# singhhp1069/charon

Hardware: AMD Instinct MI355X
Metric: verified+aggregated 3-of-4 threshold BLS sigs/sec at 1/2/4/8 MI355X (higher is better)
Workload: dtype u32 (Fp 14x28-bit limbs); 1 GPU; config2: 3-of-4, 10000 DVs x 1 attestation per GPU; parallelism=shard1, inflight_launches=3, batches_per_launch=16, rlc_group=16, rlc_chunk=8, gident=0, subgroup_batch=0, level0=passed, hw_queues=4

## Files before the change

### charon_amd/_native.py

```python
from __future__ import annotations

import ctypes
import os
import shutil
import subprocess

PKG = os.path.dirname(os.path.abspath(__file__))
ROOT = os.path.dirname(PKG)
CSRC = os.path.join(PKG, "csrc")
LIB_PATH = os.path.join(PKG, "libtbls_gpu.so")
HEADER = os.path.join(ROOT, "include", "tbls_gpu.h")
HEADERS = [HEADER, os.path.join(ROOT, "include", "tbls_ssz.h")]


def _hipcc():
    for c in ("/opt/rocm/bin/hipcc", shutil.which("hipcc") or ""):
        if c and os.path.exists(c):
            return c
    raise RuntimeError("hipcc not found: cannot build libtbls_gpu.so")


def _clangxx():
    c = "/opt/rocm/llvm/bin/clang++"
    if not os.path.exists(c):
# ... 169 lines not shown
    "tbg_submit_sets": (ctypes.c_int, [ctypes.c_void_p, ctypes.POINTER(TbgBatch), ctypes.c_void_p, ctypes.c_uint32,
                                       ctypes.POINTER(ctypes.c_uint64)]),
    "tbg_collect_sets": (ctypes.c_int, [ctypes.c_void_p, ctypes.c_uint64, ctypes.c_void_p, ctypes.c_void_p,
                                        ctypes.c_int]),
    "tbg_fetch_sets": (ctypes.c_int, [ctypes.c_void_p, ctypes.c_uint64, ctypes.c_void_p, ctypes.c_void_p]),
    "tbg_run": (ctypes.c_int, [ctypes.c_void_p, ctypes.POINTER(TbgBatch), ctypes.c_void_p, ctypes.c_void_p,
                               ctypes.c_void_p]),
    "tbg_replay": (ctypes.c_int, [ctypes.c_void_p, ctypes.c_uint64, ctypes.c_uint32, ctypes.c_void_p]),
    "tbg_replay_multi": (ctypes.c_int, [ctypes.c_void_p, ctypes.c_void_p, ctypes.c_uint32, ctypes.c_uint32,
                                        ctypes.c_void_p]),
    "tbg_fetch": (ctypes.c_int, [ctypes.c_void_p, ctypes.c_uint64, ctypes.c_void_p, ctypes.c_void_p, ctypes.c_void_p]),
    "tbg_fetch_stats": (ctypes.c_int, [ctypes.c_void_p, ctypes.c_uint64, ctypes.c_void_p]),
    "tbg_fetch_level0": (ctypes.c_int, [ctypes.c_void_p, ctypes.c_uint64, ctypes.c_void_p]),
    "tbg_fetch_fallback": (ctypes.c_int, [ctypes.c_void_p, ctypes.c_uint64, ctypes.c_void_p]),
    "tbg_fetch_subgroup": (ctypes.c_int, [ctypes.c_void_p, ctypes.c_uint64, ctypes.c_void_p]),
    "tbg_fetch_shape": (ctypes.c_int, [ctypes.c_void_p, ctypes.c_uint64, ctypes.c_void_p]),
    "tbg_host_stats": (ctypes.c_int, [ctypes.c_void_p, ctypes.c_void_p, ctypes.c_int]),
    "tbg_multi_host_stats": (ctypes.c_int, [ctypes.c_void_p, ctypes.c_void_p, ctypes.c_int]),
    "tbg_slot_bytes": (ctypes.c_int, [ctypes.c_void_p, ctypes.c_uint64, ctypes.c_void_p, ctypes.c_void_p]),
    "tbg_last_timings": (ctypes.c_int, [ctypes.c_void_p, ctypes.c_void_p]),
    "tbg_sk_to_pk": (ctypes.c_int, [ctypes.c_void_p, ctypes.c_void_p, ctypes.c_uint32, ctypes.c_void_p]),
    "tbg_sign": (ctypes.c_int, [ctypes.c_void_p, ctypes.c_void_p, ctypes.c_uint32, ctypes.c_void_p, ctypes.c_void_p,
                                ctypes.c_uint32, ctypes.c_void_p, ctypes.c_void_p]),
    "tbg_poll": (ctypes.c_int, [ctypes.c_void_p, ctypes.c_uint64]),
    "tbg_submit_group": (ctypes.c_int, [ctypes.c_void_p, ctypes.c_void_p, ctypes.c_uint32, ctypes.c_void_p]),
    "tbg_replay_profile": (ctypes.c_int, [ctypes.c_void_p, ctypes.c_uint64, ctypes.c_void_p, ctypes.c_uint32,
                                          ctypes.POINTER(ctypes.c_uint32)]),
    "tbg_replay_plan": (ctypes.c_int, [ctypes.c_void_p, ctypes.c_void_p, ctypes.c_void_p, ctypes.c_uint32,
                                       ctypes.c_void_p]),
    "tbg_multi_init": (ctypes.c_int, [ctypes.POINTER(TbgConfig), ctypes.c_void_p, ctypes.c_uint32,
# ... 21 lines not shown
    "tbg_signing_roots": (ctypes.c_int, [ctypes.c_uint32, ctypes.c_char_p, ctypes.c_uint32, ctypes.c_char_p,
                                         ctypes.c_uint32, ctypes.c_void_p, ctypes.c_void_p, ctypes.c_uint32]),
}

_lib = None


def load() -> ctypes.CDLL:
    global _lib
    if _lib is None:
        path = os.environ.get("TBG_LIB", LIB_PATH)
        if not os.path.exists(path):
            raise RuntimeError(f"{path} is missing: run __graft_entry__.build() (hipcc, gfx950)")
        lib = ctypes.CDLL(path)
        for name, (res, args) in SIGNATURES.items():
            fn = getattr(lib, name)
            fn.restype = res
            fn.argtypes = args
        _lib = lib
    return _lib
```

### charon_amd/csrc/bls_sgb.h

```cpp
#pragma once
#include "bls_pair.h"

namespace tbg {

template <class F, bool FAST>
TBG_HD Jac<F> sgb_add_g(const Jac<F>& p, const Jac<F>& q, bool& exc) {
  if constexpr (FAST) return jac_add_x(p, q, exc);
  else return jac_add(p, q);
}

template <class F, bool FAST, class L>
TBG_HD Jac<F> sgb_fold_g(L&& slice, uint32_t n_slices, bool& exc) {
  Jac<F> acc = slice(0u);
#pragma unroll 1
  for (uint32_t sl = 1; sl < n_slices; ++sl) acc = sgb_add_g<F, FAST>(acc, slice(sl), exc);
  return acc;
}

template <class F, bool FAST, class L>
TBG_HD Jac<F> sgb_running_sums_g(L&& bucket, uint32_t n_v, bool& exc) {
  Jac<F> run = jac_inf<F>(), q = run;
#pragma unroll 1
  for (int v = (int)n_v; v >= 1; --v) {
    run = sgb_add_g<F, FAST>(run, bucket((uint32_t)(v - 1)), exc);
    q = sgb_add_g<F, FAST>(q, run, exc);
  }
  return q;
}

}
```

### charon_amd/csrc/k_msm.hip

```cpp
#define TBG_ADD_DBL_INLINE 1
#ifndef TBG_SCHED_FENCE
#define TBG_SCHED_FENCE 1
#endif
#include "tbls_launch.h"
#include "bls_msm.h"
#include "bls_pair.h"
#include "bls_batchinv.h"

namespace tbg {

__global__ void __launch_bounds__(BINV_BLOCK) k_pubkey_tables(const G1A* pk, const G1A* xpk, const int32_t* status,
                                                              uint32_t n, G1A* tab) {
  const uint32_t i = blockIdx.x * blockDim.x + threadIdx.x;
  const bool in = i < n;
  const bool ok = in && status[i] == DEC_OK;
  G1A p0{fp_zero(), fp_zero()}, x0 = p0;
  if (ok) {
    p0 = pk[i];
    x0 = xpk[i];
  }
#if TBG_PK_W2
#pragma unroll 1
  for (int k = 0; k < (int)PK_TAB; ++k) {
    const G1J e = ok ? rlc_key_table_w2_entry(p0, x0, k) : jac_inf<Fp>();
// ... 212 lines not shown
  px_store(*B.batch_pt, Aff<Fp2x>{f_mul(acc.X, zi2), f_mul(acc.Y, f_mul(zi2, zi))});
}

__global__ void __launch_bounds__(2 * L0F_PAIRS) k_l0f_reduce(DevBatch B, uint32_t n_sg, uint32_t wq, uint32_t n_t) {
  __shared__ Jac<Fp2x> lds[2 * L0F_PAIRS];
  if (B.counters[CNT_L0_BAD]) return;
  const uint32_t pr = threadIdx.x >> 1, b = blockIdx.x;
  const bool qcol = b < SGB_K * wq;
  const uint32_t col = qcol ? b / wq : SGB_K, chunk = qcol ? b % wq : b - SGB_K * wq;
  const uint32_t count = qcol ? n_sg : n_sg * n_t;
  const uint32_t a0 = chunk * L0F_CHUNK + pr * L0F_PER, a1 = min(a0 + L0F_PER, count);
  Jac<Fp2x> acc = jac_inf<Fp2x>();
#pragma unroll 1
  for (uint32_t a = a0; a < a1; ++a) {
    if (qcol) {
      acc = jac_add_in<Fp2x, true>(acc, px_load(B.sgb_part[((size_t)SGB_BUCKETS * a + (size_t)SGB_V * col) * B.sgb_split]));
    } else {
      acc = jac_add_in<Fp2x, true>(acc, px_load(B.sgb_t[a]));
    }
  }
  acc = pair_tree_sum<L0F_PAIRS>(acc, lds);
  if (pr == 0) px_store(B.l0f_sum[b], acc);
}

__global__ void __launch_bounds__(2 * L0F_PAIRS) k_l0f_fold(DevBatch B, uint32_t wq, uint32_t wt) {
  TBG_URGENT();
  __shared__ Jac<Fp2x> lds[2 * L0F_PAIRS];
  if (B.counters[CNT_L0_BAD]) return;
  const uint32_t pr = threadIdx.x >> 1, col = blockIdx.x;
  const uint32_t first = col < SGB_K ? col * wq : SGB_K * wq, count = col < SGB_K ? wq : wt;
  Jac<Fp2x> acc = jac_inf<Fp2x>();
// ... 57 lines not shown
```

### charon_amd/csrc/k_sgb.hip

```cpp
#define TBG_ADD_DBL_INLINE 1
#ifndef TBG_SCHED_FENCE
#define TBG_SCHED_FENCE 1
#endif
#include "tbls_launch.h"
#include "bls_rlc.h"
#include "bls_sgb.h"

namespace tbg {

#ifndef TBG_SGB_SORT_BLOCK
#define TBG_SGB_SORT_BLOCK 256
#endif
constexpr uint32_t kSgbSortBlock = TBG_SGB_SORT_BLOCK;

__global__ void __launch_bounds__(kSgbSortBlock) k_sgb_sort(DevBatch B) {
  __shared__ uint32_t cnt[SGB_BUCKETS];
  __shared__ uint32_t off[SGB_BUCKETS + 1];
  __shared__ int8_t dig[SGB_M * SGB_K];
  const uint32_t g = blockIdx.x, t = threadIdx.x, m = B.sgb_m;
  const uint32_t i0 = g * m;
  const uint32_t n = min(m, B.n_partials - i0);
  for (uint32_t b = t; b < SGB_BUCKETS; b += kSgbSortBlock) cnt[b] = 0;
  if (t == 0) B.sgb_bad[g] = 0;
  const bool fused = l0_fused(B);
  __syncthreads();
  for (uint32_t li = t; li < n; li += kSgbSortBlock) {
    const bool ok = B.partial_status[i0 + li] == TBG_PS_NOT_VERIFIED;
    int32_t c[SGB_K];
    sgb_digits(B.sgb_seed, i0 + li, c);
    if (fused) {
      uint32_t u[4];
      l0f_digits(c, u);
      *(uint4*)(B.l0f_u + 4ull * (i0 + li)) = make_uint4(u[0], u[1], u[2], u[3]);
    }
#pragma unroll
    for (uint32_t k = 0; k < SGB_K; ++k) {
      const int32_t d = ok ? c[k] : 0;
      dig[li * SGB_K + k] = (int8_t)d;
      if (d) atomicAdd(&cnt[k * SGB_V + (uint32_t)(d < 0 ? -d : d) - 1], 1u);
    }
  }
  __syncthreads();
  if (t == 0) {
    uint32_t run = 0;
    for (uint32_t b = 0; b < SGB_BUCKETS; ++b) {
      off[b] = run;
      run += cnt[b];
    }
    off[SGB_BUCKETS] = run;
  }
// ... 5 lines not shown
  }
  __syncthreads();
  uint32_t* ent = B.sgb_ent + (size_t)m * SGB_K * g;
  for (uint32_t li = t; li < n; li += kSgbSortBlock) {
#pragma unroll 1
    for (uint32_t k = 0; k < SGB_K; ++k) {
      const int32_t d = dig[li * SGB_K + k];
      if (!d) continue;
      const uint32_t pos = atomicAdd(&cnt[k * SGB_V + (uint32_t)(d < 0 ? -d : d) - 1], 1u);
      ent[pos] = (li << 1) | (d < 0 ? 1u : 0u);
    }
  }
}

__global__ void TBG_LAUNCH_N(TBG_PAIR_WAVES) k_sgb_bucket(DevBatch B, uint32_t n_sg, uint32_t n_t) {
  const uint32_t w = (blockIdx.x * blockDim.x + threadIdx.x) >> 1;
  const uint32_t S = B.sgb_split, m = B.sgb_m;
  if (w >= n_sg * SGB_BUCKETS * S) {
    const uint32_t wt = w - n_sg * SGB_BUCKETS * S;
    if (wt >= n_sg * n_t) return;
    const uint32_t i0 = (wt / n_t) * m + (wt % n_t) * SGB_T_PER;
    const uint32_t i1 = min(min(i0 + SGB_T_PER, (wt / n_t + 1) * m), B.n_partials);
    Jac<Fp2x> acc = jac_inf<Fp2x>();
#pragma unroll 1
    for (uint32_t i = i0; i < i1; ++i) {
      if (B.partial_status[i] != TBG_PS_NOT_VERIFIED) continue;
      Aff<Fp2x> p = px_load(B.sig_aff[i]);
      p.y = f_reduce(p.y);
      acc = jac_add_aff_in(acc, p);
    }
    px_store(B.sgb_t[wt], acc);
    return;
  }
  const uint32_t g = w / (SGB_BUCKETS * S), b = (w / S) % SGB_BUCKETS, sl = w % S;
  const uint32_t* goff = B.sgb_off + (size_t)(SGB_BUCKETS + 1) * g;
  const uint32_t o0 = goff[b], n = goff[b + 1] - o0;
  const uint32_t e0 = o0 + (n * sl) / S, e1 = o0 + (n * (sl + 1)) / S;
  const uint32_t* ent = B.sgb_ent + (size_t)m * SGB_K * g;
  const G2A* sig = B.sig_aff + (size_t)m * g;
  Jac<Fp2x> acc = jac_inf<Fp2x>();
#pragma unroll 1
  for (uint32_t e = e0; e < e1; ++e) {
    const uint32_t v = ent[e];
    Aff<Fp2x> p = px_load(sig[v >> 1]);
    p.y = f_reduce(p.y);
    if (v & 1u) p.y = f_reduce(f_neg(p.y));
    acc = jac_add_aff_in(acc, p);
  }
  px_store(B.sgb_part[w], acc);
}

__device__ __forceinline__ void sgb_fail(const DevBatch& B, uint32_t g) {
  B.sgb_bad[g] = 1u;
  if (l0_fused(B)) B.counters[CNT_L0_BAD] = 1u;
}

__device__ __noinline__ Jac<Fp2x> sgb_fold_complete(const G2J* part, uint32_t S) {
  bool unused = false;
  return sgb_fold_g<Fp2x, false>([&](uint32_t sl) { return px_load(part[sl]); }, S, unused);
}

__global__ void TBG_LAUNCH_N(TBG_PAIR_WAVES) k_sgb_fold(DevBatch B, uint32_t n_sg) {
  const uint32_t w = (blockIdx.x * blockDim.x + threadIdx.x) >> 1;
  if (w >= n_sg * SGB_BUCKETS) return;
  const uint32_t S = B.sgb_split;
  G2J* part = B.sgb_part + (size_t)w * S;
  bool exc = false;
  Jac<Fp2x> acc = sgb_fold_g<Fp2x, true>([&](uint32_t sl) { return px_load(part[sl]); }, S, exc);
  if (!pair_all(!exc)) acc = sgb_fold_complete(part, S);
  px_store(part[0], acc);
}

__device__ __noinline__ Jac<Fp2x> sgb_combine_complete(const G2J* part, uint32_t S) {
  bool unused = false;
  return sgb_running_sums_g<Fp2x, false>([&](uint32_t v) { return px_load(part[(size_t)v * S]); }, SGB_V, unused);
}

__global__ void TBG_LAUNCH_N(TBG_PAIR_WAVES) k_sgb_combine(DevBatch B, uint32_t n_sg) {
  const uint32_t w = (blockIdx.x * blockDim.x + threadIdx.x) >> 1;
  if (w >= n_sg * SGB_K) return;
  const uint32_t g = w / SGB_K, k = w % SGB_K, S = B.sgb_split;
  G2J* part = B.sgb_part + ((size_t)SGB_BUCKETS * g + (size_t)SGB_V * k) * S;
  bool exc = false;
  Jac<Fp2x> q = sgb_running_sums_g<Fp2x, true>([&](uint32_t v) { return px_load(part[(size_t)v * S]); }, SGB_V, exc);
  if (!pair_all(!exc)) q = sgb_combine_complete(part, S);
  px_store(part[0], q);
}

__global__ void TBG_LAUNCH_N(TBG_PAIR_WAVES) k_sgb_test(DevBatch B, uint32_t n_sg) {
  const uint32_t w = (blockIdx.x * blockDim.x + threadIdx.x) >> 1;
  if (w >= n_sg * SGB_K) return;
  const uint32_t g = w / SGB_K, k = w % SGB_K;
  const G2J& slot = B.sgb_part[((size_t)SGB_BUCKETS * g + (size_t)SGB_V * k) * B.sgb_split];
  bool ok = true;
  if (!jac_is_inf(px_load(slot))) {
    bool exc = false;
    Jac<Fp2x> m = px_load(slot);
#pragma unroll 1
    for (int i = 62; i >= 0; --i) {
      m = jac_dbl_lo(m);
      if ((X_ABS >> i) & 1) {
        __asm__ __volatile__("" ::: "memory");
        m = jac_add_x(m, px_load(slot), exc);
      }
    }
    if (exc || jac_is_inf(m)) {
      ok = false;
    } else {
// ... 1 lines not shown
      const Jac<Fp2x> ps = g2_psi_g(px_load(slot));
      const Fp2x z1 = f_sqr(ps.Z), z2 = f_sqr(m.Z);
      ok = f_eq(f_mul(ps.X, z2), f_mul(m.X, z1)) &&
           f_eq(f_mul(f_mul(ps.Y, m.Z), z2), f_reduce(f_neg(f_mul(f_mul(m.Y, ps.Z), z1))));
    }
  }
  if (!ok && pair_par() == 0) sgb_fail(B, g);
}

void launch_subgroup_batch(const DevBatch& B, hipStream_t st) {
  if (!B.sgb) return;
  const uint32_t n_sg = sgb_groups(B.n_partials, B.sgb_m);
  if (!n_sg) return;
  TBG_KLAUNCH(k_sgb_sort, dim3(n_sg), dim3(kSgbSortBlock), st, B);
  const uint32_t n_t = l0_fused(B) ? sgb_t_slices(B.sgb_m) : 0u;
  TBG_KLAUNCH(k_sgb_bucket, grid_for(2 * n_sg * (SGB_BUCKETS * B.sgb_split + n_t)), dim3(kBlock), st, B, n_sg, n_t);
  if (B.sgb_split > 1) TBG_KLAUNCH(k_sgb_fold, grid_for(2 * n_sg * SGB_BUCKETS), dim3(kBlock), st, B, n_sg);
  TBG_KLAUNCH(k_sgb_combine, grid_for(2 * n_sg * SGB_K), dim3(kBlock), st, B, n_sg);
  TBG_KLAUNCH(k_sgb_test, grid_for(2 * n_sg * SGB_K), dim3(kBlock), st, B, n_sg);
}

}
```

### charon_amd/csrc/tbls_engine.hip

```cpp
#include <hip/hip_runtime.h>
#include <cstdio>
#include <cstdlib>
#include <cstring>
#include <cmath>
#include <functional>
#include <algorithm>
#include <atomic>
#include <chrono>
#include <mutex>
#include <new>
#include <random>
#include <thread>
#include <vector>
#include "tbls_launch.h"
#include "bls_lines.h"

using namespace tbg;

namespace tbg {
void debug_after_launch(const char* kernel, hipStream_t st) {
  static const bool on = getenv("TBG_DEBUG_SYNC") && getenv("TBG_DEBUG_SYNC")[0] == '1';
  if (!on) return;
  hipEvent_t a;
  (void)hipEventCreate(&a);
// ... 642 lines not shown
  size_t w_bf = sec(l0 ? 4ull * 3 * 4 * NL : 0);
  size_t w_gf = sec(l0 ? 4ull * 3 * 4 * NL * grp_f_entries(ng) : 0);
  const bool gm = TBG_GMSM && G != 0;
  size_t w_gmoff = sec(gm ? 4ull * (GM_BUCKETS + 1) * ng : 0);
  size_t w_gment = sec(gm ? 64ull * np : 0);
  size_t w_gmpart = sec(gm ? sizeof(G2J) * GM_BUCKETS * (size_t)ng : 0);
  size_t w_gmlead = sec(gm ? 4ull * ng : 0);
  size_t w_gmlist = sec(gm ? 4ull * np : 0);
  size_t w_gmhist = sec(gm ? 4ull * 256 : 0);
  size_t w_gmorder = sec(gm ? 4ull * GM_BUCKETS * ng : 0);
  uint32_t sgb_m = SGB_M;
  const bool sgb = np >= SGB_MIN_PARTIALS && c->sgb_mode != TBG_SGB_OFF &&
                   (sgb_plan(c->nonsub_ema, sgb_m) || c->sgb_mode == TBG_SGB_ON);
  const uint32_t sgb_split = sgb_split_for(sgb_m);
  const size_t n_sg = sgb ? sgb_groups(np, sgb_m) : 0;
  size_t w_sgoff = sec(4ull * (SGB_BUCKETS + 1) * n_sg);
  size_t w_sgent = sec(4ull * sgb_m * SGB_K * n_sg);
  size_t w_sgpart = sec(sizeof(G2J) * SGB_BUCKETS * sgb_split * n_sg);
  size_t w_sgbad = sec(4ull * n_sg);
  const bool fused = l0 && sgb && TBG_PK_W2;
  const bool msm = l0 && !fused;
  size_t w_mr = sec(msm ? 8ull * np : 0);
  size_t w_moff = sec(msm ? 4ull * (MSM_BUCKETS + 1) : 0);
  size_t w_mcur = sec(msm ? 4ull * MSM_BUCKETS : 0);
  size_t w_ment = sec(msm ? 16ull * np : 0);
  size_t w_mbkt = sec(msm ? sizeof(G2J) * (size_t)MSM_BUCKETS : 0);
  size_t w_mpart = sec(msm ? sizeof(G2J) * (size_t)MSM_BUCKETS * MSM_SPLIT : 0);
  size_t w_msum = sec(msm ? sizeof(G2J) * (size_t)MSM_SUM_ENTRIES : 0);
  size_t w_sgt = sec(fused ? sizeof(G2J) * sgb_t_slices(sgb_m) * n_sg : 0);
  size_t w_l0fsum = sec(fused ? sizeof(G2J) * (size_t)l0f_sum_entries((uint32_t)n_sg, sgb_m) : 0);
  size_t w_l0fu = sec(fused ? 16ull * np : 0);
  size_t w_aacc = sec(op != TBG_OP_VERIFY ? sizeof(G2J) * (size_t)nd : 0);
  size_t w_alist = sec(op != TBG_OP_VERIFY ? 4ull * nd : 0);
// ... 218 lines not shown
  B.batch_f = (uint32_t*)(dw + w_bf);
  B.grp_f = (uint32_t*)(dw + w_gf);
  B.gm_off = (uint32_t*)(dw + w_gmoff);
  B.gm_ent = (uint32_t*)(dw + w_gment);
  B.gm_part = (G2J*)(dw + w_gmpart);
  B.gm_lead = (uint32_t*)(dw + w_gmlead);
  B.gm_list = (uint32_t*)(dw + w_gmlist);
  B.gm_hist = (uint32_t*)(dw + w_gmhist);
  B.gm_order = (uint32_t*)(dw + w_gmorder);
  B.sgb = sgb ? 1u : 0u;
  B.sgb_m = sgb_m;
  B.sgb_split = sgb_split;
  B.sgb_off = (uint32_t*)(dw + w_sgoff);
  B.sgb_ent = (uint32_t*)(dw + w_sgent);
  B.sgb_part = (G2J*)(dw + w_sgpart);
  B.sgb_bad = (uint32_t*)(dw + w_sgbad);
  B.sgb_t = (G2J*)(dw + w_sgt);
  B.l0f_sum = (G2J*)(dw + w_l0fsum);
  B.l0f_u = (uint32_t*)(dw + w_l0fu);
  B.agg_acc = (G2J*)(dw + w_aacc);
  B.agg_list = (uint32_t*)(dw + w_alist);

  hipStream_t st = s->st;
  if (hipStreamWaitEvent(st, c->keys_ready, 0) != hipSuccess ||
      hipMemcpyAsync(s->d_in, s->h_in, in_bytes, hipMemcpyHostToDevice, st) != hipSuccess)
    return release(TBG_E_DEVICE);
  rc = launch_chain(c, *s, B, s->ev);
  if (rc != TBG_OK) return release(rc);
  if (hipMemcpyAsync(s->h_out, dw + w_out, out_bytes, hipMemcpyDeviceToHost, st) != hipSuccess ||
      hipEventRecord(s->done, st) != hipSuccess)
// ... 356 lines not shown
int tbg_fetch_subgroup(tbg_ctx* c, tbg_ticket t, uint32_t* out3) {
  if (!c || !out3) return TBG_E_INVALID_ARG;
  std::lock_guard<std::mutex> lk(c->mu);
  Slot* s = find_ticket(c, t, false, nullptr);
  if (!s) return TBG_E_TICKET;
  HIP_TRY(hipSetDevice(c->device));
  out3[0] = out3[1] = out3[2] = 0;
  if (!s->last.sgb) return TBG_OK;
  out3[2] = s->last.sgb_m;
  const uint32_t n_sg = sgb_groups(s->last.n_partials, s->last.sgb_m);
  std::vector<uint32_t> bad(n_sg);
  HIP_TRY(hipMemcpyAsync(bad.data(), s->last.sgb_bad, 4ull * n_sg, hipMemcpyDeviceToHost, s->st));
  HIP_TRY(hipStreamSynchronize(s->st));
  out3[0] = n_sg;
  for (uint32_t g = 0; g < n_sg; ++g) out3[1] += bad[g] ? 1u : 0u;
  return TBG_OK;
}

int tbg_host_stats(tbg_ctx* c, uint64_t* out8, int reset) {
  if (!c || !out8) return TBG_E_INVALID_ARG;
  for (int k = 0; k < 8; ++k) out8[k] = reset ? c->host[k].exchange(0) : c->host[k].load();
  return TBG_OK;
}

int tbg_slot_bytes(tbg_ctx* c, tbg_ticket t, uint64_t* device_bytes, uint64_t* pinned_bytes) {
  if (!c || !device_bytes || !pinned_bytes) return TBG_E_INVALID_ARG;
  std::lock_guard<std::mutex> lk(c->mu);
  Slot* s = find_ticket(c, t, false, nullptr);
  if (!s) return TBG_E_TICKET;
  *device_bytes = (uint64_t)s->d_in_cap + (uint64_t)s->d_work_cap;
// ... 305 lines not shown
```

### charon_amd/csrc/tbls_launch.h

```cpp
#pragma once
#include <hip/hip_runtime.h>
#include "bls_curve.h"
#include "bls_lines.h"
#include "../../include/tbls_gpu.h"

namespace tbg {

constexpr int kBlock = 64;
#ifndef TBG_PK_W2
#define TBG_PK_W2 1
#endif
constexpr uint32_t PK_TAB = TBG_PK_W2 ? 8u : 2u;
#ifndef TBG_REPLAY_SHAPE
#define TBG_REPLAY_SHAPE 1
#endif
#ifndef TBG_L0_SHAPE
#define TBG_L0_SHAPE 1
#endif
#ifndef TBG_L0_SHAPE_WIDE
#define TBG_L0_SHAPE_WIDE 1
#endif
#ifndef TBG_FB_WINDOW
#define TBG_FB_WINDOW 32768u
#endif
// ... 83 lines not shown
  uint32_t* grp_f;
  uint32_t* gm_off;
  uint32_t* gm_ent;
  G2J* gm_part;
  uint32_t* gm_lead;
  uint32_t* gm_list;
  uint32_t* gm_hist;
  uint32_t* gm_order;
  uint32_t sgb;
  uint32_t sgb_m;
  uint32_t sgb_split;
  uint32_t sgb_seed[8];
  uint32_t* sgb_off;
  uint32_t* sgb_ent;
  G2J* sgb_part;
  uint32_t* sgb_bad;
  G2J* sgb_t;
  G2J* l0f_sum;
  uint32_t* l0f_u;
  G2J* agg_acc;
  uint32_t* agg_list;
  int32_t* partial_status;
  int32_t* duty_status;
  uint8_t* agg;
  uint32_t sets;
  uint32_t n_sets;
  const uint32_t* duty_set;
  int32_t* set_status;
};
enum SetTail : int { SET_BAD = 0, SET_ANY = 1, SET_TAIL = 2 };
// ... 12 lines not shown
#endif
#ifndef TBG_SGB_SPLIT
#define TBG_SGB_SPLIT 4
#endif
constexpr uint32_t SGB_M = TBG_SGB_M;
constexpr uint32_t SGB_M_MIN = 64;
constexpr uint32_t SGB_K = 18;
constexpr uint32_t SGB_V = 6;
constexpr uint32_t SGB_BUCKETS = SGB_K * SGB_V;
constexpr uint32_t SGB_SPLIT = TBG_SGB_SPLIT;
constexpr uint32_t SGB_MIN_PARTIALS = 2 * SGB_M;
TBG_HD uint32_t sgb_groups(uint32_t n_partials, uint32_t m) { return (n_partials + m - 1) / m; }
TBG_HD uint32_t sgb_split_for(uint32_t m) {
  const uint32_t s = SGB_SPLIT * m / SGB_M;
  return s ? s : 1u;
}
TBG_HD bool l0_fused(const DevBatch& B) {
  return TBG_PK_W2 && B.rlc_batch && B.rlc_group && B.sgb && B.n_partials;
}
constexpr uint32_t SGB_T_PER = 32;
TBG_HD uint32_t sgb_t_slices(uint32_t m) { return m / SGB_T_PER; }
constexpr uint32_t L0F_COLS = SGB_K + 1;
constexpr uint32_t L0F_PAIRS = 128, L0F_PER = 4;
constexpr uint32_t L0F_CHUNK = L0F_PAIRS * L0F_PER;
TBG_HD uint32_t l0f_q_chunks(uint32_t n_sg) { return (n_sg + L0F_CHUNK - 1) / L0F_CHUNK; }
TBG_HD uint32_t l0f_t_chunks(uint32_t n_sg, uint32_t m) { return (n_sg * sgb_t_slices(m) + L0F_CHUNK - 1) / L0F_CHUNK; }
TBG_HD uint32_t l0f_sum_entries(uint32_t n_sg, uint32_t m) {
  return SGB_K * l0f_q_chunks(n_sg) + l0f_t_chunks(n_sg, m) + L0F_COLS;
}
constexpr uint32_t L0_TREE_FAN = 4;
// ... 102 lines not shown
```

### charon_amd/engine.py

```python
from __future__ import annotations

import ctypes
import itertools
from dataclasses import dataclass

import numpy as np

from . import _native

PS_INVALID, PS_VALID, PS_NOT_VERIFIED = 0, 1, 2
PS_ERR_FLAGS, PS_ERR_FIELD, PS_ERR_CURVE, PS_ERR_SUBGROUP, PS_ERR_IDENTITY, PS_ERR_PUBKEY = -1, -2, -3, -4, -5, -6
DS_OK, DS_NOT_AGGREGATED = 0, 1
DS_INSUFFICIENT, DS_INSUFFICIENT_VALID = -20, -21
DS_AGG_TOO_FEW, DS_AGG_DUPLICATE_ID, DS_AGG_IDENTITY, DS_DECODE = -22, -23, -24, -25
SS_ERROR, SS_INVALID, SS_VALID = 30, 31, 32
OP_VERIFY, OP_AGGREGATE, OP_VERIFY_AGGREGATE = 1, 2, 3
NO_PUBKEY = 0xFFFFFFFF
TIMING_KEYS = ["decode", "hash", "combine", "h_lines", "verify", "lagrange", "aggregate", "total"]
VERIFY_RLC, VERIFY_EACH = 0, 1
RLC_L0_AUTO, RLC_L0_ON, RLC_L0_OFF = 0, 1, 2
GIDENT_OFF, GIDENT_L3, GIDENT_CHUNKS = 0, 1, 2
SGB_AUTO, SGB_ON, SGB_OFF = 0, 1, 2
EXPRESS_OFF = 0xFFFFFFFF
L0_NOT_RUN, L0_PASSED, L0_FAILED = 0, 1, 2
HOST_STAT_KEYS = ["submits", "partials_submitted", "pack_ns", "enqueue_ns", "collects", "partials_collected",
                  "gather_ns", "wait_ns"]
MULTI_HOST_STAT_KEYS = ["submits", "partials", "build_ns", "submit_wall_ns", "collects", "collect_wall_ns"] + \
    ["ctx_" + k for k in HOST_STAT_KEYS] + ["contexts", "reserved"]
E_PENDING = -6
E_INVALID_ARG, E_TICKET = -1, -7


class EngineError(RuntimeError):
    pass


def _ptr(a):
# ... 222 lines not shown
        out = np.zeros(4, dtype=np.uint32)
        self._check(self._lib.tbg_fetch_stats(self._h, ticket, _ptr(out)), "tbg_fetch_stats")
        return dict(zip(["groups", "duty_checks", "partial_checks", "group_size"], out.tolist()))

    def fallback(self, ticket) -> dict:
        out = np.zeros(8, dtype=np.uint32)
        self._check(self._lib.tbg_fetch_fallback(self._h, ticket, _ptr(out)), "tbg_fetch_fallback")
        return dict(zip(["groups", "group_searches", "chunks", "chunk_searches", "duty_searches", "partial_checks",
                         "group_size", "level0"], out.tolist()))

    def shape(self, ticket) -> dict:
        out = np.zeros(4, dtype=np.uint32)
        self._check(self._lib.tbg_fetch_shape(self._h, ticket, _ptr(out)), "tbg_fetch_shape")
        return dict(zip(["group", "chunk", "level0", "chunks"], out.tolist()))

    def subgroup(self, ticket) -> dict:
        out = np.zeros(3, dtype=np.uint32)
        self._check(self._lib.tbg_fetch_subgroup(self._h, ticket, _ptr(out)), "tbg_fetch_subgroup")
        return dict(zip(["groups", "failed", "group_size"], out.tolist()))

    def host_stats(self, reset=False) -> dict:
        out = np.zeros(8, dtype=np.uint64)
        self._check(self._lib.tbg_host_stats(self._h, _ptr(out), 1 if reset else 0), "tbg_host_stats")
        return dict(zip(HOST_STAT_KEYS, out.tolist()))

    def slot_bytes(self, ticket) -> tuple:
        dev, pin = ctypes.c_uint64(), ctypes.c_uint64()
        self._check(self._lib.tbg_slot_bytes(self._h, ticket, ctypes.byref(dev), ctypes.byref(pin)), "tbg_slot_bytes")
        return dev.value, pin.value

    def level0(self, ticket) -> int:
        st = ctypes.c_int32(0)
        self._check(self._lib.tbg_fetch_level0(self._h, ticket, ctypes.byref(st)), "tbg_fetch_level0")
        return st.value
# ... 183 lines not shown
```

### include/tbls_gpu.h

```cpp
#ifndef TBLS_GPU_H
#define TBLS_GPU_H

#include <stddef.h>
#include <stdint.h>

#ifdef __cplusplus
extern "C" {
#endif

#define TBG_OK 0
#define TBG_E_INVALID_ARG (-1)
#define TBG_E_DEVICE (-2)
#define TBG_E_OOM (-3)
#define TBG_E_NO_DEVICE (-4)
#define TBG_E_BUSY (-5)
#define TBG_E_PENDING (-6)
#define TBG_E_TICKET (-7)

#define TBG_PS_INVALID 0
#define TBG_PS_VALID 1
#define TBG_PS_NOT_VERIFIED 2
#define TBG_PS_ERR_FLAGS (-1)
#define TBG_PS_ERR_FIELD (-2)
#define TBG_PS_ERR_CURVE (-3)
// ... 110 lines not shown

int tbg_replay(tbg_ctx* ctx, tbg_ticket ticket, uint32_t iters, float* ms8);
int tbg_replay_multi(tbg_ctx* ctx, const tbg_ticket* tickets, uint32_t n_tickets, uint32_t iters, float* ms8);
int tbg_replay_plan(tbg_ctx* ctx, const tbg_ticket* tickets, const uint32_t* n_parts, uint32_t n_launches, float* ms8);
int tbg_fetch(tbg_ctx* ctx, tbg_ticket ticket, int32_t* partial_status, int32_t* duty_status, uint8_t* agg96);
typedef struct {
  char name[64];
  float ms;
} tbg_kernel_time;
int tbg_replay_profile(tbg_ctx* ctx, tbg_ticket ticket, tbg_kernel_time* out, uint32_t max_entries,
                       uint32_t* n_entries);
int tbg_fetch_stats(tbg_ctx* ctx, tbg_ticket ticket, uint32_t* out4);
int tbg_fetch_level0(tbg_ctx* ctx, tbg_ticket ticket, int32_t* state);
int tbg_fetch_fallback(tbg_ctx* ctx, tbg_ticket ticket, uint32_t* out8);
int tbg_fetch_subgroup(tbg_ctx* ctx, tbg_ticket ticket, uint32_t* out3);
int tbg_fetch_shape(tbg_ctx* ctx, tbg_ticket ticket, uint32_t* out4);
int tbg_host_stats(tbg_ctx* ctx, uint64_t* out8, int reset);
int tbg_slot_bytes(tbg_ctx* ctx, tbg_ticket ticket, uint64_t* device_bytes, uint64_t* pinned_bytes);

int tbg_sum_pubkeys(tbg_ctx* ctx, const uint32_t* pubkey_ids, const uint32_t* off, uint32_t n_sets, uint8_t* out48,
                    int32_t* status);
int tbg_sum_sigs(tbg_ctx* ctx, const uint8_t* sigs96, const uint32_t* off, uint32_t n_sets, uint8_t* out96,
                 int32_t* status, int32_t* sig_status);
int tbg_fast_aggregate_verify(tbg_ctx* ctx, const uint32_t* pubkey_ids, const uint32_t* key_off, uint32_t n_sets,
                              const uint8_t* msgs, const uint32_t* msg_off, const uint8_t* sigs96, int32_t* status);

int tbg_sk_to_pk(tbg_ctx* ctx, const uint8_t* sk32, uint32_t n, uint8_t* pk48);
int tbg_sign(tbg_ctx* ctx, const uint8_t* sk32, uint32_t n, const uint8_t* msgs, const uint32_t* msg_off,
             uint32_t n_msgs, const uint32_t* item_msg, uint8_t* sig96);

// ... 20 lines not shown
```

Before: 3.454 million DV-duties/s (n verifies + 1 aggregate each).

## Add paired-digit subgroup bucket schedule with count-ranked bucket dispatch

For subgroup sizes of at least 256, signed digits are combined in pairs into joint buckets, which roughly halves the number of bucket entries per partial. Bucket workers are dispatched in order of bucket occupancy so waves get similar amounts of work. A fold kernel rebuilds the per-digit bucket sums from the pair buckets. The cost is more buckets, extra fold additions, and more sort logic. A query that reports which schedule ran is also added.

Measured after the change: 3.573 million DV-duties/s (n verifies + 1 aggregate each), median of 6. 1.03x the previous value.

```diff
diff --git a/charon_amd/_native.py b/charon_amd/_native.py
--- a/charon_amd/_native.py
+++ b/charon_amd/_native.py
@@ -207,6 +207,7 @@
     "tbg_fetch_level0": (ctypes.c_int, [ctypes.c_void_p, ctypes.c_uint64, ctypes.c_void_p]),
     "tbg_fetch_fallback": (ctypes.c_int, [ctypes.c_void_p, ctypes.c_uint64, ctypes.c_void_p]),
     "tbg_fetch_subgroup": (ctypes.c_int, [ctypes.c_void_p, ctypes.c_uint64, ctypes.c_void_p]),
+    "tbg_fetch_subgroup_schedule": (ctypes.c_int, [ctypes.c_void_p, ctypes.c_uint64, ctypes.c_void_p]),
     "tbg_fetch_shape": (ctypes.c_int, [ctypes.c_void_p, ctypes.c_uint64, ctypes.c_void_p]),
     "tbg_host_stats": (ctypes.c_int, [ctypes.c_void_p, ctypes.c_void_p, ctypes.c_int]),
     "tbg_multi_host_stats": (ctypes.c_int, [ctypes.c_void_p, ctypes.c_void_p, ctypes.c_int]),
@@ -258,7 +259,11 @@
             raise RuntimeError(f"{path} is missing: run __graft_entry__.build() (hipcc, gfx950)")
         lib = ctypes.CDLL(path)
         for name, (res, args) in SIGNATURES.items():
-            fn = getattr(lib, name)
+            fn = getattr(lib, name, None)
+            if fn is None:
+                if path == LIB_PATH:
+                    raise RuntimeError(f"{path} does not export {name}: rebuild it (__graft_entry__.build())")
+                continue
             fn.restype = res
             fn.argtypes = args
         _lib = lib
diff --git a/charon_amd/csrc/bls_sgb.h b/charon_amd/csrc/bls_sgb.h
--- a/charon_amd/csrc/bls_sgb.h
+++ b/charon_amd/csrc/bls_sgb.h
@@ -28,4 +28,38 @@
   return q;
 }
 
+constexpr uint32_t SGBP_V = 6;
+constexpr uint32_t SGBP_ROW = 2 * SGBP_V + 1;
+constexpr uint32_t SGBP_B = SGBP_V + SGBP_V * SGBP_ROW;
+constexpr uint32_t SGBP_SUMS = 2 * SGBP_V;
+constexpr uint32_t SGBP_NONE = 0xFFu;
+TBG_HD uint32_t sgb_pair_index(uint32_t a, int32_t b) {
+  return a ? SGBP_V + (a - 1) * SGBP_ROW + (uint32_t)(b + (int32_t)SGBP_V) : (uint32_t)b - 1;
 }
+TBG_HD uint32_t sgb_pair_code(int32_t c0, int32_t c1) {
+  if (!c0 && !c1) return SGBP_NONE;
+  const bool neg = c0 < 0 || (!c0 && c1 < 0);
+  return sgb_pair_index((uint32_t)(neg ? -c0 : c0), neg ? -c1 : c1) | (neg ? 0x80u : 0u);
+}
+template <class F, bool FAST, class L>
+TBG_HD Jac<F> sgb_pair_sum_g(L&& bucket, uint32_t j, bool& exc) {
+  Jac<F> acc = jac_inf<F>();
+#pragma unroll 1
+  for (uint32_t t = 0; t < SGBP_ROW; ++t) {
+    uint32_t idx;
+    bool neg = false;
+    if (j < SGBP_V) {
+      idx = sgb_pair_index(j + 1, (int32_t)t - (int32_t)SGBP_V);
+    } else {
+      const int32_t v = (int32_t)(j - SGBP_V) + 1;
+      neg = t > SGBP_V;
+      idx = t == 0 ? sgb_pair_index(0, v) : sgb_pair_index(neg ? t - SGBP_V : t, neg ? -v : v);
+    }
+    Jac<F> x = bucket(idx);
+    if (neg) x = jac_neg(x);
+    acc = sgb_add_g<F, FAST>(acc, x, exc);
+  }
+  return acc;
+}
+
+}
diff --git a/charon_amd/csrc/k_msm.hip b/charon_amd/csrc/k_msm.hip
--- a/charon_amd/csrc/k_msm.hip
+++ b/charon_amd/csrc/k_msm.hip
@@ -250,7 +250,7 @@
 #pragma unroll 1
   for (uint32_t a = a0; a < a1; ++a) {
     if (qcol) {
-      acc = jac_add_in<Fp2x, true>(acc, px_load(B.sgb_part[((size_t)SGB_BUCKETS * a + (size_t)SGB_V * col) * B.sgb_split]));
+      acc = jac_add_in<Fp2x, true>(acc, px_load(B.sgb_part[sgb_q_slot(B, a, col)]));
     } else {
       acc = jac_add_in<Fp2x, true>(acc, px_load(B.sgb_t[a]));
     }
diff --git a/charon_amd/csrc/k_sgb.hip b/charon_amd/csrc/k_sgb.hip
--- a/charon_amd/csrc/k_sgb.hip
+++ b/charon_amd/csrc/k_sgb.hip
@@ -13,14 +13,51 @@
 #endif
 constexpr uint32_t kSgbSortBlock = TBG_SGB_SORT_BLOCK;
 
-__global__ void __launch_bounds__(kSgbSortBlock) k_sgb_sort(DevBatch B) {
-  __shared__ uint32_t cnt[SGB_BUCKETS];
-  __shared__ uint32_t off[SGB_BUCKETS + 1];
-  __shared__ int8_t dig[SGB_M * SGB_K];
+static_assert(SGBP_B == SGB_PB && SGBP_V == SGB_V && SGBP_SUMS * SGB_PAIRS == SGB_BUCKETS, "bls_sgb.h's pair layout");
+static_assert((kSgbSortBlock & (kSgbSortBlock - 1)) == 0, "sgb_block_scan: a power of two");
+constexpr uint32_t SGB_RANK_KEYS = 256;
+
+template <uint32_t N>
+__device__ __forceinline__ void sgb_block_scan(uint32_t* a, uint32_t* tmp) {
+  constexpr uint32_t PER = (N + kSgbSortBlock - 1) / kSgbSortBlock;
+  const uint32_t t = threadIdx.x, b0 = t * PER;
+  uint32_t sum = 0;
+  for (uint32_t j = 0; j < PER; ++j)
+    if (b0 + j < N) sum += a[b0 + j];
+  tmp[t] = sum;
+  __syncthreads();
+  for (uint32_t d = 1; d < kSgbSortBlock; d <<= 1) {
+    const uint32_t x = t >= d ? tmp[t - d] : 0u;
+    __syncthreads();
+    tmp[t] += x;
+    __syncthreads();
+  }
+  uint32_t run = tmp[t] - sum;
+  for (uint32_t j = 0; j < PER; ++j)
+    if (b0 + j < N) {
+      const uint32_t x = a[b0 + j];
+      a[b0 + j] = run;
+      run += x;
+    }
+  if (t == kSgbSortBlock - 1) a[N] = tmp[t];
+  __syncthreads();
+}
+
+__device__ __forceinline__ void sgb_sort_paired(const DevBatch& B, uint8_t* lds) {
+  uint8_t* code = lds;
+  uint32_t* cnt = (uint32_t*)(lds + SGB_M * SGB_PAIRS);
+  uint32_t* hist = cnt + SGB_PBUCKETS + 1;
+  uint32_t* tmp = hist + SGB_RANK_KEYS + 1;
+  uint8_t* key = (uint8_t*)(tmp + kSgbSortBlock);
+  static_assert((SGB_M * SGB_PAIRS) % 4 == 0 &&
+                    SGB_M * SGB_PAIRS + 4 * (SGB_PBUCKETS + 1 + SGB_RANK_KEYS + 1 + kSgbSortBlock) + SGB_PBUCKETS <=
+                        SGB_M * SGB_K,
+                "the paired sort's arrays fit the digit array");
   const uint32_t g = blockIdx.x, t = threadIdx.x, m = B.sgb_m;
   const uint32_t i0 = g * m;
   const uint32_t n = min(m, B.n_partials - i0);
-  for (uint32_t b = t; b < SGB_BUCKETS; b += kSgbSortBlock) cnt[b] = 0;
+  for (uint32_t b = t; b < SGB_PBUCKETS; b += kSgbSortBlock) cnt[b] = 0;
+  for (uint32_t b = t; b < SGB_RANK_KEYS; b += kSgbSortBlock) hist[b] = 0;
   if (t == 0) B.sgb_bad[g] = 0;
   const bool fused = l0_fused(B);
   __syncthreads();
@@ -34,6 +71,65 @@
       *(uint4*)(B.l0f_u + 4ull * (i0 + li)) = make_uint4(u[0], u[1], u[2], u[3]);
     }
 #pragma unroll
+    for (uint32_t p = 0; p < SGB_PAIRS; ++p) {
+      const uint32_t cd = ok ? sgb_pair_code(c[2 * p], c[2 * p + 1]) : SGBP_NONE;
+      code[li * SGB_PAIRS + p] = (uint8_t)cd;
+      if (cd != SGBP_NONE) atomicAdd(&cnt[p * SGB_PB + (cd & 0x7Fu)], 1u);
+    }
+  }
+  __syncthreads();
+  for (uint32_t b = t; b < SGB_PBUCKETS; b += kSgbSortBlock) {
+    const uint32_t k = SGB_RANK_KEYS - 1 - min(cnt[b], SGB_RANK_KEYS - 1);
+    key[b] = (uint8_t)k;
+    atomicAdd(&hist[k], 1u);
+  }
+  __syncthreads();
+  sgb_block_scan<SGB_PBUCKETS>(cnt, tmp);
+  sgb_block_scan<SGB_RANK_KEYS>(hist, tmp);
+  uint32_t* goff = B.sgb_off + (size_t)(SGB_PBUCKETS + 1) * g;
+  uint32_t* rank = B.sgb_rank + (size_t)SGB_PBUCKETS * g;
+  for (uint32_t b = t; b <= SGB_PBUCKETS; b += kSgbSortBlock) {
+    goff[b] = cnt[b];
+    if (b < SGB_PBUCKETS) rank[atomicAdd(&hist[key[b]], 1u)] = b;
+  }
+  __syncthreads();
+  uint32_t* ent = B.sgb_ent + (size_t)sgb_ent_stride(m) * g;
+  for (uint32_t li = t; li < n; li += kSgbSortBlock) {
+#pragma unroll 1
+    for (uint32_t p = 0; p < SGB_PAIRS; ++p) {
+      const uint32_t cd = code[li * SGB_PAIRS + p];
+      if (cd == SGBP_NONE) continue;
+      const uint32_t pos = atomicAdd(&cnt[p * SGB_PB + (cd & 0x7Fu)], 1u);
+      ent[pos] = (li << 1) | (cd >> 7);
+    }
+  }
+}
+
+__global__ void __launch_bounds__(kSgbSortBlock) k_sgb_sort(DevBatch B) {
+  __shared__ uint32_t cnt[SGB_BUCKETS];
+  __shared__ uint32_t off[SGB_BUCKETS + 1];
+  __shared__ __attribute__((aligned(16))) int8_t dig[SGB_M * SGB_K];
+  if (sgb_paired(B.sgb_m)) {
+    sgb_sort_paired(B, (uint8_t*)dig);
+    return;
+  }
+  const uint32_t g = blockIdx.x, t = threadIdx.x, m = B.sgb_m;
+  const uint32_t i0 = g * m;
+  const uint32_t n = min(m, B.n_partials - i0);
+  for (uint32_t b = t; b < SGB_BUCKETS; b += kSgbSortBlock) cnt[b] = 0;
+  if (t == 0) B.sgb_bad[g] = 0;
+  const bool fused = l0_fused(B);
+  __syncthreads();
+  for (uint32_t li = t; li < n; li += kSgbSortBlock) {
+    const bool ok = B.partial_status[i0 + li] == TBG_PS_NOT_VERIFIED;
+    int32_t c[SGB_K];
+    sgb_digits(B.sgb_seed, i0 + li, c);
+    if (fused) {
+      uint32_t u[4];
+      l0f_digits(c, u);
+      *(uint4*)(B.l0f_u + 4ull * (i0 + li)) = make_uint4(u[0], u[1], u[2], u[3]);
+    }
+#pragma unroll
     for (uint32_t k = 0; k < SGB_K; ++k) {
       const int32_t d = ok ? c[k] : 0;
       dig[li * SGB_K + k] = (int8_t)d;
@@ -69,10 +165,13 @@
 }
 
 __global__ void TBG_LAUNCH_N(TBG_PAIR_WAVES) k_sgb_bucket(DevBatch B, uint32_t n_sg, uint32_t n_t) {
-  const uint32_t w = (blockIdx.x * blockDim.x + threadIdx.x) >> 1;
+  uint32_t w = (blockIdx.x * blockDim.x + threadIdx.x) >> 1;
   const uint32_t S = B.sgb_split, m = B.sgb_m;
-  if (w >= n_sg * SGB_BUCKETS * S) {
-    const uint32_t wt = w - n_sg * SGB_BUCKETS * S;
+  const bool paired = sgb_paired(m);
+  const uint32_t per_g = paired ? SGB_PRANK : SGB_BUCKETS * S;
+  const bool is_t = paired ? w < n_sg * n_t : w >= n_sg * per_g;
+  if (is_t) {
+    const uint32_t wt = paired ? w : w - n_sg * per_g;
     if (wt >= n_sg * n_t) return;
     const uint32_t i0 = (wt / n_t) * m + (wt % n_t) * SGB_T_PER;
     const uint32_t i1 = min(min(i0 + SGB_T_PER, (wt / n_t + 1) * m), B.n_partials);
@@ -87,11 +186,28 @@
     px_store(B.sgb_t[wt], acc);
     return;
   }
-  const uint32_t g = w / (SGB_BUCKETS * S), b = (w / S) % SGB_BUCKETS, sl = w % S;
-  const uint32_t* goff = B.sgb_off + (size_t)(SGB_BUCKETS + 1) * g;
-  const uint32_t o0 = goff[b], n = goff[b + 1] - o0;
-  const uint32_t e0 = o0 + (n * sl) / S, e1 = o0 + (n * (sl + 1)) / S;
-  const uint32_t* ent = B.sgb_ent + (size_t)m * SGB_K * g;
+  if (paired) w -= n_sg * n_t;
+  if (w >= n_sg * per_g) return;
+  const uint32_t g = w / per_g;
+  uint32_t e0, e1;
+  size_t out;
+  if (paired) {
+    const uint32_t r = w % SGB_PRANK;
+    if (r >= SGB_PBUCKETS) return;
+    const uint32_t b = B.sgb_rank[(size_t)SGB_PBUCKETS * g + r];
+    const uint32_t* goff = B.sgb_off + (size_t)(SGB_PBUCKETS + 1) * g;
+    e0 = goff[b];
+    e1 = goff[b + 1];
+    out = (size_t)sgb_part_stride(m) * g + b;
+  } else {
+    const uint32_t b = (w / S) % SGB_BUCKETS, sl = w % S;
+    const uint32_t* goff = B.sgb_off + (size_t)(SGB_BUCKETS + 1) * g;
+    const uint32_t o0 = goff[b], n = goff[b + 1] - o0;
+    e0 = o0 + (n * sl) / S;
+    e1 = o0 + (n * (sl + 1)) / S;
+    out = w;
+  }
+  const uint32_t* ent = B.sgb_ent + (size_t)sgb_ent_stride(m) * g;
   const G2A* sig = B.sig_aff + (size_t)m * g;
   Jac<Fp2x> acc = jac_inf<Fp2x>();
 #pragma unroll 1
@@ -102,7 +218,7 @@
     if (v & 1u) p.y = f_reduce(f_neg(p.y));
     acc = jac_add_aff_in(acc, p);
   }
-  px_store(B.sgb_part[w], acc);
+  px_store(B.sgb_part[out], acc);
 }
 
 __device__ __forceinline__ void sgb_fail(const DevBatch& B, uint32_t g) {
@@ -115,9 +231,24 @@
   return sgb_fold_g<Fp2x, false>([&](uint32_t sl) { return px_load(part[sl]); }, S, unused);
 }
 
+__device__ __noinline__ Jac<Fp2x> sgb_pair_sum_complete(const G2J* bk, uint32_t j) {
+  bool unused = false;
+  return sgb_pair_sum_g<Fp2x, false>([&](uint32_t idx) { return px_load(bk[idx]); }, j, unused);
+}
+
 __global__ void TBG_LAUNCH_N(TBG_PAIR_WAVES) k_sgb_fold(DevBatch B, uint32_t n_sg) {
   const uint32_t w = (blockIdx.x * blockDim.x + threadIdx.x) >> 1;
   if (w >= n_sg * SGB_BUCKETS) return;
+  if (sgb_paired(B.sgb_m)) {
+    const uint32_t g = w / SGB_BUCKETS, p = (w % SGB_BUCKETS) / SGBP_SUMS, j = w % SGBP_SUMS;
+    G2J* grp = B.sgb_part + (size_t)sgb_part_stride(B.sgb_m) * g;
+    const G2J* bk = grp + (size_t)SGB_PB * p;
+    bool exc = false;
+    Jac<Fp2x> acc = sgb_pair_sum_g<Fp2x, true>([&](uint32_t idx) { return px_load(bk[idx]); }, j, exc);
+    if (!pair_all(!exc)) acc = sgb_pair_sum_complete(bk, j);
+    px_store(grp[SGB_PBUCKETS + w % SGB_BUCKETS], acc);
+    return;
+  }
   const uint32_t S = B.sgb_split;
   G2J* part = B.sgb_part + (size_t)w * S;
   bool exc = false;
@@ -134,8 +265,8 @@
 __global__ void TBG_LAUNCH_N(TBG_PAIR_WAVES) k_sgb_combine(DevBatch B, uint32_t n_sg) {
   const uint32_t w = (blockIdx.x * blockDim.x + threadIdx.x) >> 1;
   if (w >= n_sg * SGB_K) return;
-  const uint32_t g = w / SGB_K, k = w % SGB_K, S = B.sgb_split;
-  G2J* part = B.sgb_part + ((size_t)SGB_BUCKETS * g + (size_t)SGB_V * k) * S;
+  const uint32_t g = w / SGB_K, k = w % SGB_K, S = sgb_paired(B.sgb_m) ? 1u : B.sgb_split;
+  G2J* part = B.sgb_part + sgb_q_slot(B, g, k);
   bool exc = false;
   Jac<Fp2x> q = sgb_running_sums_g<Fp2x, true>([&](uint32_t v) { return px_load(part[(size_t)v * S]); }, SGB_V, exc);
   if (!pair_all(!exc)) q = sgb_combine_complete(part, S);
@@ -146,7 +277,7 @@
   const uint32_t w = (blockIdx.x * blockDim.x + threadIdx.x) >> 1;
   if (w >= n_sg * SGB_K) return;
   const uint32_t g = w / SGB_K, k = w % SGB_K;
-  const G2J& slot = B.sgb_part[((size_t)SGB_BUCKETS * g + (size_t)SGB_V * k) * B.sgb_split];
+  const G2J& slot = B.sgb_part[sgb_q_slot(B, g, k)];
   bool ok = true;
   if (!jac_is_inf(px_load(slot))) {
     bool exc = false;
@@ -178,8 +309,10 @@
   if (!n_sg) return;
   TBG_KLAUNCH(k_sgb_sort, dim3(n_sg), dim3(kSgbSortBlock), st, B);
   const uint32_t n_t = l0_fused(B) ? sgb_t_slices(B.sgb_m) : 0u;
-  TBG_KLAUNCH(k_sgb_bucket, grid_for(2 * n_sg * (SGB_BUCKETS * B.sgb_split + n_t)), dim3(kBlock), st, B, n_sg, n_t);
-  if (B.sgb_split > 1) TBG_KLAUNCH(k_sgb_fold, grid_for(2 * n_sg * SGB_BUCKETS), dim3(kBlock), st, B, n_sg);
+  const bool paired = sgb_paired(B.sgb_m);
+  const uint32_t per_g = paired ? SGB_PRANK : SGB_BUCKETS * B.sgb_split;
+  TBG_KLAUNCH(k_sgb_bucket, grid_for(2 * n_sg * (per_g + n_t)), dim3(kBlock), st, B, n_sg, n_t);
+  if (paired || B.sgb_split > 1) TBG_KLAUNCH(k_sgb_fold, grid_for(2 * n_sg * SGB_BUCKETS), dim3(kBlock), st, B, n_sg);
   TBG_KLAUNCH(k_sgb_combine, grid_for(2 * n_sg * SGB_K), dim3(kBlock), st, B, n_sg);
   TBG_KLAUNCH(k_sgb_test, grid_for(2 * n_sg * SGB_K), dim3(kBlock), st, B, n_sg);
 }
diff --git a/charon_amd/csrc/tbls_engine.hip b/charon_amd/csrc/tbls_engine.hip
--- a/charon_amd/csrc/tbls_engine.hip
+++ b/charon_amd/csrc/tbls_engine.hip
@@ -680,9 +680,10 @@
                    (sgb_plan(c->nonsub_ema, sgb_m) || c->sgb_mode == TBG_SGB_ON);
   const uint32_t sgb_split = sgb_split_for(sgb_m);
   const size_t n_sg = sgb ? sgb_groups(np, sgb_m) : 0;
-  size_t w_sgoff = sec(4ull * (SGB_BUCKETS + 1) * n_sg);
-  size_t w_sgent = sec(4ull * sgb_m * SGB_K * n_sg);
-  size_t w_sgpart = sec(sizeof(G2J) * SGB_BUCKETS * sgb_split * n_sg);
+  size_t w_sgoff = sec(4ull * sgb_off_stride(sgb_m) * n_sg);
+  size_t w_sgent = sec(4ull * sgb_ent_stride(sgb_m) * n_sg);
+  size_t w_sgpart = sec(sizeof(G2J) * sgb_part_stride(sgb_m) * n_sg);
+  size_t w_sgrank = sec(sgb_paired(sgb_m) ? 4ull * SGB_PBUCKETS * n_sg : 0);
   size_t w_sgbad = sec(4ull * n_sg);
   const bool fused = l0 && sgb && TBG_PK_W2;
   const bool msm = l0 && !fused;
@@ -931,6 +932,7 @@
   B.sgb_off = (uint32_t*)(dw + w_sgoff);
   B.sgb_ent = (uint32_t*)(dw + w_sgent);
   B.sgb_part = (G2J*)(dw + w_sgpart);
+  B.sgb_rank = (uint32_t*)(dw + w_sgrank);
   B.sgb_bad = (uint32_t*)(dw + w_sgbad);
   B.sgb_t = (G2J*)(dw + w_sgt);
   B.l0f_sum = (G2J*)(dw + w_l0fsum);
@@ -1317,6 +1319,17 @@
   HIP_TRY(hipStreamSynchronize(s->st));
   out3[0] = n_sg;
   for (uint32_t g = 0; g < n_sg; ++g) out3[1] += bad[g] ? 1u : 0u;
+  return TBG_OK;
+}
+
+int tbg_fetch_subgroup_schedule(tbg_ctx* c, tbg_ticket t, uint32_t* out1) {
+  if (!c || !out1) return TBG_E_INVALID_ARG;
+  std::lock_guard<std::mutex> lk(c->mu);
+  Slot* s = find_ticket(c, t, false, nullptr);
+  if (!s) return TBG_E_TICKET;
+  *out1 = !s->last.sgb                 ? (uint32_t)TBG_SGB_SCHED_NONE
+          : sgb_paired(s->last.sgb_m) ? (uint32_t)TBG_SGB_SCHED_PAIRED
+                                      : (uint32_t)TBG_SGB_SCHED_CLASSIC;
   return TBG_OK;
 }
 
diff --git a/charon_amd/csrc/tbls_launch.h b/charon_amd/csrc/tbls_launch.h
--- a/charon_amd/csrc/tbls_launch.h
+++ b/charon_amd/csrc/tbls_launch.h
@@ -121,6 +121,7 @@
   uint32_t* sgb_off;
   uint32_t* sgb_ent;
   G2J* sgb_part;
+  uint32_t* sgb_rank;
   uint32_t* sgb_bad;
   G2J* sgb_t;
   G2J* l0f_sum;
@@ -163,6 +164,21 @@
 TBG_HD uint32_t sgb_split_for(uint32_t m) {
   const uint32_t s = SGB_SPLIT * m / SGB_M;
   return s ? s : 1u;
+}
+constexpr uint32_t SGB_PAIR_M = 256;
+constexpr uint32_t SGB_PAIRS = SGB_K / 2;
+constexpr uint32_t SGB_PB = SGB_V + SGB_V * (2 * SGB_V + 1);
+constexpr uint32_t SGB_PBUCKETS = SGB_PAIRS * SGB_PB;
+constexpr uint32_t SGB_PRANK = (SGB_PBUCKETS + 31) / 32 * 32;
+TBG_HD bool sgb_paired(uint32_t m) { return m >= SGB_PAIR_M; }
+TBG_HD uint32_t sgb_off_stride(uint32_t m) { return (sgb_paired(m) ? SGB_PBUCKETS : SGB_BUCKETS) + 1; }
+TBG_HD uint32_t sgb_ent_stride(uint32_t m) { return m * (sgb_paired(m) ? SGB_PAIRS : SGB_K); }
+TBG_HD uint32_t sgb_part_stride(uint32_t m) {
+  return sgb_paired(m) ? SGB_PBUCKETS + SGB_BUCKETS : SGB_BUCKETS * sgb_split_for(m);
+}
+TBG_HD size_t sgb_q_slot(const DevBatch& B, uint32_t g, uint32_t k) {
+  return (size_t)sgb_part_stride(B.sgb_m) * g +
+         (sgb_paired(B.sgb_m) ? SGB_PBUCKETS + SGB_V * k : SGB_V * k * B.sgb_split);
 }
 TBG_HD bool l0_fused(const DevBatch& B) {
   return TBG_PK_W2 && B.rlc_batch && B.rlc_group && B.sgb && B.n_partials;
diff --git a/charon_amd/engine.py b/charon_amd/engine.py
--- a/charon_amd/engine.py
+++ b/charon_amd/engine.py
@@ -21,6 +21,7 @@
 RLC_L0_AUTO, RLC_L0_ON, RLC_L0_OFF = 0, 1, 2
 GIDENT_OFF, GIDENT_L3, GIDENT_CHUNKS = 0, 1, 2
 SGB_AUTO, SGB_ON, SGB_OFF = 0, 1, 2
+SGB_SCHEDULES = ("none", "classic", "paired")
 EXPRESS_OFF = 0xFFFFFFFF
 L0_NOT_RUN, L0_PASSED, L0_FAILED = 0, 1, 2
 HOST_STAT_KEYS = ["submits", "partials_submitted", "pack_ns", "enqueue_ns", "collects", "partials_collected",
@@ -273,10 +274,16 @@
         self._check(self._lib.tbg_fetch_shape(self._h, ticket, _ptr(out)), "tbg_fetch_shape")
         return dict(zip(["group", "chunk", "level0", "chunks"], out.tolist()))
 
-    def subgroup(self, ticket) -> dict:
+    def subgroup(self, ticket, schedule: bool = False) -> dict:
         out = np.zeros(3, dtype=np.uint32)
         self._check(self._lib.tbg_fetch_subgroup(self._h, ticket, _ptr(out)), "tbg_fetch_subgroup")
-        return dict(zip(["groups", "failed", "group_size"], out.tolist()))
+        res = dict(zip(["groups", "failed", "group_size"], out.tolist()))
+        if schedule:
+            sched = np.zeros(1, dtype=np.uint32)
+            self._check(self._lib.tbg_fetch_subgroup_schedule(self._h, ticket, _ptr(sched)),
+                        "tbg_fetch_subgroup_schedule")
+            res["schedule"] = SGB_SCHEDULES[int(sched[0])]
+        return res
 
     def host_stats(self, reset=False) -> dict:
         out = np.zeros(8, dtype=np.uint64)
diff --git a/include/tbls_gpu.h b/include/tbls_gpu.h
--- a/include/tbls_gpu.h
+++ b/include/tbls_gpu.h
@@ -148,6 +148,10 @@
 int tbg_fetch_level0(tbg_ctx* ctx, tbg_ticket ticket, int32_t* state);
 int tbg_fetch_fallback(tbg_ctx* ctx, tbg_ticket ticket, uint32_t* out8);
 int tbg_fetch_subgroup(tbg_ctx* ctx, tbg_ticket ticket, uint32_t* out3);
+#define TBG_SGB_SCHED_NONE 0
+#define TBG_SGB_SCHED_CLASSIC 1
+#define TBG_SGB_SCHED_PAIRED 2
+int tbg_fetch_subgroup_schedule(tbg_ctx* ctx, tbg_ticket ticket, uint32_t* out1);
 int tbg_fetch_shape(tbg_ctx* ctx, tbg_ticket ticket, uint32_t* out4);
 int tbg_host_stats(tbg_ctx* ctx, uint64_t* out8, int reset);
 int tbg_slot_bytes(tbg_ctx* ctx, tbg_ticket ticket, uint64_t* device_bytes, uint64_t* pinned_bytes);
```
